# JoeyOL/PytorchDistributed

Measured on AMD Instinct MI355X. Metric: images/sec (whole node) ResNet-50 DDP at 1/2/4/8 MI355X; scaling efficiency, higher is better.
Workload: dtype bf16; 1 GPU; model=resnet50, global_batch=640, per_gpu_batch=640, image_size=224, parallelism=dp1, optimizer=SGD(momentum=0.9, wd=5e-5), fp32 master weights

## Files before the change

### csrc/bindings.cpp

```cpp
#include <torch/extension.h>
#include <c10/hip/HIPStream.h>

#include <map>
#include <mutex>
#include <c10/core/DeviceGuard.h>

#include "pda_kernels.h"
#include "runtime.h"

namespace pda_rt {
void bind_runtime(pybind11::module& m);
}
namespace pda_comm {
void bind_comm(pybind11::module& m);
}

namespace py = pybind11;
using at::Tensor;

namespace {

#define CHECK_HIP_OK(expr)                                                                  \
  do {                                                                                      \
    hipError_t _e = (expr);                                                                 \
// ... 432 lines not shown
  TORCH_CHECK(table.dim() == 3 && table.size(1) == 2 && table.size(2) == C && table.is_contiguous());
  if (relu) {
    TORCH_CHECK(bits.has_value() || ss.has_value(), "relu backward needs the bit mask or scale/shift");
    if (bits.has_value()) {
      check_gpu(*bits, "bits");
      TORCH_CHECK(bits->scalar_type() == at::kByte && bits->is_contiguous() && bits->numel() * 8 == x.numel());
    } else {
      check_f32(*ss, "ss");
      TORCH_CHECK(ss->numel() == 2 * C);
    }
  }
  check_f32(mean, "mean");
  check_f32(invstd, "invstd");
  const float* gf;
  const pda::bf16_t* gb;
  bn_param_ptrs(gamma, &gf, &gb, C);
  c10::DeviceGuard g(x.device());
  Tensor dx = at::empty_like(x);
  Tensor dres = want_dres ? at::empty_like(x) : Tensor();
  const auto pdt = gamma.has_value() ? gamma->scalar_type() : at::kFloat;
  Tensor dgamma = dgamma_out.has_value() ? *dgamma_out : at::empty({C}, x.options().dtype(pdt));
  Tensor dbeta = dbeta_out.has_value() ? *dbeta_out : at::empty({C}, x.options().dtype(pdt));
  TORCH_CHECK(dgamma.numel() == C && dbeta.numel() == C && dgamma.scalar_type() == pdt && dbeta.scalar_type() == pdt);
  const bool pb = pdt == at::kBFloat16;
  Tensor coef = at::empty({3 * C}, x.options().dtype(at::kFloat));
  CHECK_HIP_OK(pda::bn_bwd_table(bp(dy), bp(x), (relu && bits.has_value()) ? bits->data_ptr<uint8_t>() : nullptr,
                                 (relu && !bits.has_value()) ? ss->data_ptr<float>() : nullptr, M, C,
                                 mean.data_ptr<float>(), invstd.data_ptr<float>(), gf, gb, relu, bpm(dx),
                                 want_dres ? bpm(dres) : nullptr, pb ? nullptr : dgamma.data_ptr<float>(),
                                 pb ? bpm(dgamma) : nullptr, pb ? nullptr : dbeta.data_ptr<float>(),
                                 pb ? bpm(dbeta) : nullptr, table.data_ptr<float>(), (int)table.size(0),
                                 coef.data_ptr<float>(), stream_of(x)));
  return {dx, dres, dgamma, dbeta};
}

std::vector<Tensor> maxpool_fwd(Tensor x, int64_t k, int64_t s, int64_t pad) {
  check_bf16(x, "x");
  TORCH_CHECK(x.dim() == 4, "x must be [N,H,W,C]");
  const int N = x.size(0), H = x.size(1), W = x.size(2), C = x.size(3);
  TORCH_CHECK(C % 8 == 0 && k * k <= 255);
  const int P = (H + 2 * pad - k) / s + 1, Q = (W + 2 * pad - k) / s + 1;
  c10::DeviceGuard g(x.device());
  Tensor y = at::empty({N, P, Q, C}, x.options());
  Tensor idx = at::empty({N, P, Q, C}, x.options().dtype(at::kByte));
  CHECK_HIP_OK(pda::maxpool2d_fwd(bp(x), bpm(y), idx.data_ptr<uint8_t>(), N, H, W, C, P, Q, k, s, pad, stream_of(x)));
  return {y, idx};
}

std::vector<Tensor> bn_relu_maxpool_fwd(Tensor x, Tensor table, Tensor shift, c10::optional<Tensor> gamma,
                                        c10::optional<Tensor> beta, Tensor running_mean, Tensor running_var,
                                        c10::optional<Tensor> num_batches, double momentum, double eps, int64_t k,
                                        int64_t s, int64_t pad) {
  check_bf16(x, "x");
  TORCH_CHECK(x.dim() == 4 && x.is_contiguous(), "x must be a contiguous [N,H,W,C] tensor");
  const int N = x.size(0), H = x.size(1), W = x.size(2), C = x.size(3);
  TORCH_CHECK(C % 8 == 0 && C <= 2048 && k * k <= 255);
  check_f32(table, "table");
  check_f32(shift, "shift");
  check_f32(running_mean, "running_mean");
  check_f32(running_var, "running_var");
  TORCH_CHECK(shift.numel() == C && table.numel() % (2 * C) == 0 && table.numel() > 0 && table.is_contiguous(),
              "table must be [R, 2, C]");
  const int P = (H + 2 * pad - k) / s + 1, Q = (W + 2 * pad - k) / s + 1;
  c10::DeviceGuard g(x.device());
  auto fo = x.options().dtype(at::kFloat);
  Tensor stats = at::empty({4, C}, fo);
// ... 1176 lines not shown
  TORCH_CHECK(x.dim() == 4 && x.is_contiguous());
  const int N = x.size(0), HW = x.size(1) * x.size(2), C = x.size(3);
  c10::DeviceGuard g(x.device());
  Tensor y = at::empty({N, C}, x.options());
  CHECK_HIP_OK(pda::avgpool_f32_fwd(x.data_ptr<float>(), y.data_ptr<float>(), N, HW, C, stream_of(x)));
  return y;
}

Tensor avgpool_f32_bwd(Tensor dy, int64_t H, int64_t W) {
  check_f32(dy, "dy");
  TORCH_CHECK(dy.dim() == 2 && dy.is_contiguous());
  const int N = dy.size(0), C = dy.size(1);
  c10::DeviceGuard g(dy.device());
  Tensor dx = at::empty({N, H, W, C}, dy.options());
  CHECK_HIP_OK(pda::avgpool_f32_bwd(dy.data_ptr<float>(), dx.data_ptr<float>(), N, H * W, C, stream_of(dy)));
  return dx;
}

PYBIND11_MODULE(_C, m) {
  m.def("stream_create", &stream_create, py::arg("device"), py::arg("priority"));
  m.def("stream_priority_range", &stream_priority_range, py::arg("device"));
  m.def("stream_create_cumask", &stream_create_cumask, py::arg("device"), py::arg("ncu"), py::arg("invert") = false);
  m.doc() = "pytorchdistributed_amd native layer: CDNA4 HIP kernels + C++ runtime";
  m.def("sgd_step", &sgd_step);
  m.def("adam_step", &adam_step);
  m.def("grad_norm", &grad_norm);
  m.def("cast_scale", &cast_scale);
  m.def("ce_fwd", &ce_fwd);
  m.def("ce_bwd", &ce_bwd);
  m.def("bn_fwd_train", &bn_fwd_train);
  m.def("bn_fwd_eval", &bn_fwd_eval);
  m.def("bn_bwd", &bn_bwd);
  m.def("bn_bwd_table", &bn_bwd_table);
  m.def("set_bn_bwd_fused_max_c", &set_bn_bwd_fused_max_c);
  m.def("set_dgrad_stream", [](int64_t m) { pda::set_dgrad_stream((int)m); });
  m.def("set_fwd_stream", [](int64_t m) { pda::set_fwd_stream((int)m); });
  m.def("set_attn_bwd_fused", [](int64_t m) { pda::attention_bwd_fused_mode() = (int)m; });
  m.def("attn_bwd_fused_mode", []() { return (int64_t)pda::attention_bwd_fused_mode(); });
  m.def("bn_bwd_fused_max_c", []() { return bn_bwd_fused_max_c(); });
  m.def("maxpool_fwd", &maxpool_fwd);
  m.def("bn_relu_maxpool_fwd", &bn_relu_maxpool_fwd);
  m.def("stem_pool_bn_bwd", &stem_pool_bn_bwd);
  m.def("stem_pool_bn_bwd_ok", &stem_pool_bn_bwd_ok);
  m.def("stem_s2d", &stem_s2d);
  m.def("maxpool_bwd", &maxpool_bwd);
  m.def("avgpool_fwd", &avgpool_fwd);
  m.def("avgpool_bwd", &avgpool_bwd);
  m.def("fill_random", &fill_random);
  m.def("fill_randint", &fill_randint);
  m.def("gemm", &gemm);
  m.def("gemm_act", &gemm_act);
  m.def("gemm_wgrad_db", &gemm_wgrad_db);
  m.def("gemm_pp_lab", &gemm_pp_lab);
  m.def("set_gemm_paths", &pda::set_gemm_paths,
        "force a GEMM kernel path: wide=-1 env default, 0 off, 1 auto, 2 force", pybind11::arg("wide"));
  m.def("set_gemm_pp", &pda::set_gemm_pp,
        "pipelined 256x256 kernel for plain wide GEMMs: -1 env default (PDA_GEMM_PP), 0 off, 1 on",
        pybind11::arg("on"));
  m.def("set_splitk_fixup", &pda::set_splitk_fixup,
        "split-K weight gradients reduced by the GEMM's last split per tile: -1 env default (PDA_SPLITK_FIXUP, "
        "off), 0 separate reduce launch, 1 on",
        pybind11::arg("on"));
  m.def("conv_fwd", &conv_fwd, py::arg("x"), py::arg("w"), py::arg("stride"), py::arg("pad"), py::arg("dil"),
        py::arg("bias") = py::none(), py::arg("relu") = false, py::arg("out_f32") = false);
  m.def("split_bf16", &split_bf16, py::arg("x"), py::arg("nseg"), py::arg("lo_mask"), py::arg("stack"));
  m.def("bn_f32_fwd_train", &bn_f32_fwd_train);
// ... 67 lines not shown
```

### csrc/include/pda_kernels.h

```cpp
#pragma once
#include <hip/hip_runtime.h>
#include <stdint.h>

namespace pda {
typedef uint16_t bf16_t;

struct AttnParams {
  const bf16_t *q, *k, *v;
  bf16_t* o;
  float* lse;
  int64_t q_sb, q_st, q_sh, k_sb, k_st, k_sh, v_sb, v_st, v_sh, o_sb, o_st, o_sh;
  int B, T, Hq, Hkv, D, causal;
  float scale;
  const float *rope_cos, *rope_sin;
  const bf16_t* dout;
  int64_t do_sb, do_st, do_sh;
  float* delta;
  bf16_t *dq, *dk, *dv;
  int64_t dq_sb, dq_st, dq_sh, dk_sb, dk_st, dk_sh, dv_sb, dv_st, dv_sh;
  float* dkv_part;
  float* dq_acc;
};

constexpr int kXgmiMaxRanks = 8;
// ... 138 lines not shown
                     void* C, bool c_f32, int64_t ldc, int64_t M, int64_t N, int64_t K, const void* bias,
                     bool bias_f32, bool relu, float* slab, bool allow_split, hipStream_t st);
hipError_t gemm_bf16_wgrad_db(const bf16_t* dy, int64_t ld_dy, const bf16_t* x, int64_t ld_x, void* dw, bool dw_f32,
                              int64_t ldc, int64_t M, int64_t N, int64_t K, void* db, bool db_bf16, float* slab,
                              float* rs_scratch, hipStream_t st, int* db_done);
hipError_t gemm_bf16_act(const bf16_t* A, bool a_kmajor, int64_t lda, const bf16_t* B, bool b_kmajor, int64_t ldb,
                         bf16_t* C, int64_t ldc, int64_t M, int64_t N, int64_t K, const void* bias, bool bias_f32,
                         int act, bf16_t* act_aux, hipStream_t st);
int64_t conv_slab_floats(int mode, int N, int H, int W, int C, int Cout, int R, int S, int P, int Q);
hipError_t conv2d_fwd(const bf16_t* x, const bf16_t* w, void* y, bool y_f32, int N, int H, int W, int C, int Cout,
                      int R, int S, int P, int Q, int stride, int pad, int dil, const void* bias, bool bias_f32,
                      bool relu, float* stats, const float* stats_shift, int stats_rows, hipStream_t st);
bool conv_dgrad_needs_wt(int R, int S, int stride, int pad);
bool conv_dgrad_1x1_wt(int R, int S, int stride, int pad, int C, int Cout);
struct BnBwdStats {
  const bf16_t* z;
  const float* ss;
  const uint8_t* bits;
  const float* mean;
  float* table;
  int rows;
  const bf16_t* z2;
  const float* mean2;
  float* table2;
};
hipError_t conv2d_dgrad(const bf16_t* dy, const bf16_t* w, const bf16_t* wt, void* dx, bool dx_f32, int N, int H, int W,
                        int C, int Cout, int R, int S, int P, int Q, int stride, int pad, int dil, const bf16_t* addend,
                        const uint8_t* addend_bits, hipStream_t st, const BnBwdStats* bst = nullptr);
void set_dgrad_stream(int mode);
void set_fwd_stream(int mode);
hipError_t conv2d_wgrad(const bf16_t* dy, const bf16_t* x, void* dw, bool dw_f32, int N, int H, int W, int C,
                        int Cout, int R, int S, int P, int Q, int stride, int pad, int dil, float* slab,
                        hipStream_t st);
hipError_t conv_weight_transpose(const bf16_t* w, bf16_t* wt, int Cout, int R, int S, int Cin, int stride, int pad,
                                 int dil, hipStream_t st);


hipError_t act_fwd(const void* x, void* y, bool bf16, int64_t n, int op, hipStream_t st);
hipError_t act_bwd(const void* dy, const void* ref, void* dx, bool bf16, int64_t n, int op, hipStream_t st);
hipError_t swiglu_fwd(const void* gu, void* y, bool bf16, int64_t rows, int64_t F, hipStream_t st);
hipError_t swiglu_bwd(const void* dy, const void* gu, void* dgu, bool bf16, int64_t rows, int64_t F, hipStream_t st);
hipError_t colsum_unaligned(const void* x, bool bf16, float* out, int64_t rows, int64_t cols, hipStream_t st);

hipError_t gemm_pp_lab(const bf16_t* A, bool a_kmajor, int64_t lda, const bf16_t* B, bool b_kmajor, int64_t ldb,
                       bf16_t* C, int64_t ldc, int64_t M, int64_t N, int64_t K, const bf16_t* bias, int variant,
                       hipStream_t st);

hipError_t simt_gemm(const void* A, int a_dt, int64_t sam, int64_t sak, const void* B, int b_dt, int64_t sbk,
                     int64_t sbn, void* C, int c_dt, int64_t scm, int64_t scn, int64_t M, int64_t N, int64_t K,
                     const float* bias, bool relu, float beta, hipStream_t st);

hipError_t add_rownorm_fwd(const bf16_t* x, const bf16_t* r, const bf16_t* gamma, const bf16_t* beta, bf16_t* h,
                           bf16_t* y, int64_t rows, int64_t D, float eps, bool rms, hipStream_t st,
                           float* mean = nullptr, float* rstd = nullptr);
hipError_t rownorm_fwd(const void* x, bool x_bf16, const void* gamma, const void* beta, bool p_bf16, void* y,
                       float* mean, float* rstd, int64_t rows, int64_t D, float eps, bool rms, hipStream_t st);
hipError_t rownorm_bwd(const void* dy, const void* x, bool x_bf16, const void* gamma, bool p_bf16, const float* mean,
                       const float* rstd, void* dx, void* dgamma, void* dbeta, bool dparam_bf16, int64_t rows,
                       int64_t D, bool rms, float* ws, hipStream_t st, const void* addend = nullptr);
hipError_t colsum(const void* x, bool bf16, void* out, bool out_bf16, int64_t rows, int64_t cols, float* ws,
                  hipStream_t st);
int64_t colreduce_ws_floats(int64_t rows, int64_t D, int nout);

hipError_t attention_fwd(const AttnParams& p, hipStream_t st);
hipError_t attention_bwd(const AttnParams& p, hipStream_t st);
int64_t attention_bwd_ws_floats(int B, int T, int Hq, int Hkv, int D, bool rope);
// ... 72 lines not shown
```

### csrc/kernels/batchnorm.hip

```cpp
#include "pda_common.h"
#include "pda_kernels.h"

#include <cstdlib>

namespace pda {
namespace {

constexpr int kThreads = 256;
constexpr int kMaxC = 2048;

struct BnGeom {
  int cv;
  int cols;
  int rpi;
  int gy;
  int64_t rpb;
  int nrb;
};

BnGeom bn_geom(int64_t M, int64_t C) {
  BnGeom g;
  g.cv = (int)(C / 8);
  if (g.cv >= kThreads) {
    g.cols = kThreads;
// ... 1128 lines not shown
  int ns = lds_tables_forced() ? 0 : wave_sets((int)(C / 8));
  if (ns == 3 || ns > 4) ns = 0;
  const int grid = ns ? wave_grid(M * C / 8) : ew_grid(M * C / 8);
  const size_t lds = 5 * (size_t)C * sizeof(float);
#define BWD_APPLY(MK, DR)                                                                                        \
  do {                                                                                                           \
    if (ns == 1) bn_bwd_apply_wave_kernel<MK, DR, 1><<<grid, kThreads, 0, st>>>(dy, x, y, ss, M, (int)C, coef, dx, dres); \
    else if (ns == 2) bn_bwd_apply_wave_kernel<MK, DR, 2><<<grid, kThreads, 0, st>>>(dy, x, y, ss, M, (int)C, coef, dx, dres); \
    else if (ns == 4) bn_bwd_apply_wave_kernel<MK, DR, 4><<<grid, kThreads, 0, st>>>(dy, x, y, ss, M, (int)C, coef, dx, dres); \
    else bn_bwd_apply_kernel<MK, DR><<<grid, kThreads, lds, st>>>(dy, x, y, ss, M, (int)C, coef, dx, dres);     \
  } while (0)
  if (mask == 0) { if (dres) BWD_APPLY(0, true); else BWD_APPLY(0, false); }
  else if (mask == 1) { if (dres) BWD_APPLY(1, true); else BWD_APPLY(1, false); }
  else if (mask == 2) { if (dres) BWD_APPLY(2, true); else BWD_APPLY(2, false); }
  else { if (dres) BWD_APPLY(3, true); else BWD_APPLY(3, false); }
#undef BWD_APPLY
  return hipGetLastError();
}

hipError_t bn_bwd_table(const bf16_t* dy, const bf16_t* x, const uint8_t* relu_bits, const float* ss, int64_t M,
                        int64_t C, const float* save_mean, const float* save_invstd, const float* gamma_f,
                        const bf16_t* gamma_b, bool relu, bf16_t* dx, bf16_t* dres, float* dgamma_f, bf16_t* dgamma_b,
                        float* dbeta_f, bf16_t* dbeta_b, float* table, int rows, float* coef, hipStream_t st) {
  if (C > kMaxC || C % 8 || rows < 1 || !table) return hipErrorInvalidValue;
  if (relu && !ss && !relu_bits) return hipErrorInvalidValue;
  bn_bwd_finalize_kernel<true><<<(unsigned)((C + 63) / 64), kFinThreads, 0, st>>>(
      table, rows, M, (int)C, save_mean, save_invstd, gamma_f, gamma_b, dgamma_f, dgamma_b, dbeta_f, dbeta_b, coef);
  PDA_CHECK_HIP(hipGetLastError());
  const int mask = !relu ? 0 : (relu_bits ? 3 : 2);
  const bf16_t* y = mask == 3 ? reinterpret_cast<const bf16_t*>(relu_bits) : nullptr;
  return bwd_apply(dy, x, y, ss, M, C, coef, dx, dres, mask, st);
}

bool bn_bwd_dual_ok(int64_t C) {
  if (C % 8 || C > kMaxC || lds_tables_forced()) return false;
  const int ns = wave_sets((int)(C / 8));
  return ns == 1 || ns == 2;
}

hipError_t bn_bwd_dual(const bf16_t* dy, const uint8_t* relu_bits, int64_t M, int64_t C, const BnBwdSide& a,
                       const BnBwdSide& b, hipStream_t st) {
  if (!bn_bwd_dual_ok(C) || !relu_bits) return hipErrorInvalidValue;
  BnGeom g = bn_geom(M, C);
  float* coef = a.ws + 2 * (int64_t)g.nrb * C;
  float* coef2 = b.ws + 2 * (int64_t)g.nrb * C;
  const bool tables = a.table && b.table;
  if ((a.table != nullptr) != (b.table != nullptr) || (tables && (a.rows < 1 || b.rows < 1))) return hipErrorInvalidValue;
  if (!tables) {
    bn_bwd_reduce_dual_kernel<<<dim3(g.nrb, g.gy), kThreads, 0, st>>>(dy, a.x, b.x, relu_bits, a.mean, b.mean, M,
                                                                     (int)C, g.cols, g.rpi, g.rpb, a.ws, b.ws);
    PDA_CHECK_HIP(hipGetLastError());
  }
  const BnBwdSide* sides[2] = {&a, &b};
  float* coefs[2] = {coef, coef2};
  for (int i = 0; i < 2; ++i) {
    const BnBwdSide& p = *sides[i];
    if (tables)
      bn_bwd_finalize_kernel<true><<<(unsigned)((C + 63) / 64), kFinThreads, 0, st>>>(
          p.table, p.rows, M, (int)C, p.mean, p.invstd, p.gamma_f, p.gamma_b, p.dgamma_f, p.dgamma_b, p.dbeta_f,
          p.dbeta_b, coefs[i]);
    else
      bn_bwd_finalize_kernel<false><<<(unsigned)((C + 63) / 64), kFinThreads, 0, st>>>(
          p.ws, g.nrb, M, (int)C, p.mean, p.invstd, p.gamma_f, p.gamma_b, p.dgamma_f, p.dgamma_b, p.dbeta_f,
          p.dbeta_b, coefs[i]);
    PDA_CHECK_HIP(hipGetLastError());
  }
// ... 38 lines not shown
```

### pytorchdistributed_amd/ops/conv.py

```python
from __future__ import annotations

import os

import torch
import torch.nn.functional as F

from .._native import C
from ..parallel.flat import grad_target
from . import streams as _streams
from .grad_join import MaskedGrad


_SIDE_1X1 = os.environ.get("PDA_WGRAD_SIDE_1X1", "1") == "1"


def _ref_conv(x, w, stride, padding, dilation, bias=None):
    y = F.conv2d(x.permute(0, 3, 1, 2), w.permute(0, 3, 1, 2), bias, stride, padding, dilation)
    return y.permute(0, 2, 3, 1).contiguous()


class _Conv2dFn(torch.autograd.Function):
    @staticmethod
    def forward(ctx, x, w, bias, stride, padding, dilation, relu, join, bnb=None):
        x = x.contiguous()
        w = w.contiguous()
        y = C().conv_fwd(x, w, stride, padding, dilation, bias, relu)
        ctx.save_for_backward(x, w, y if relu else None)
        ctx.cfg = (stride, padding, dilation, relu, bias is not None)
        ctx.wparam = w
        ctx.join = join
        ctx.bnb = bnb
        return y

    @staticmethod
    def backward(ctx, dy):
        return _Conv2dFn._backward(ctx, dy)

    @staticmethod
    def _backward(ctx, dy):
        x, w, y = ctx.saved_tensors
        stride, padding, dilation, relu, has_bias = ctx.cfg
        dy = dy.contiguous()
        if relu:
            dy = C().relu_bwd(dy, y)
        dx = dw = db = None
        if ctx.needs_input_grad[0]:
            join = ctx.join
            if join is not None and not join.is_last():
                join.stash(C().conv_dgrad(dy, w, x.shape[1], x.shape[2], stride, padding, dilation, None))
            else:
                bnb = getattr(ctx, "bnb", None)
                join_last = join is not None and join.is_last()
                addend = join.take() if join is not None else None
                bits = None
                if isinstance(addend, MaskedGrad):
                    addend, bits = addend.grad, addend.bits
                kw = {}
                if bnb is not None and bnb.usable(join_last, join is not None, stride, addend) and \
                        bnb.z.shape == x.shape:
                    kw = bnb.dgrad_kwargs()
                dx = C().conv_dgrad(dy, w, x.shape[1], x.shape[2], stride, padding, dilation, addend, bits, **kw)
                if kw:
                    bnb.mark_filled(dx)
        ctx.bnb = None
        if ctx.needs_input_grad[1]:
            target = grad_target(ctx.wparam)
            args = (dy, x, w.shape[1], w.shape[2], stride, padding, dilation, w.dtype == torch.float32, target)
            if target is not None and _streams.side_ok(ctx.wparam) and (_SIDE_1X1 or w.shape[1] * w.shape[2] > 1):
                with _streams.wgrad_stream(dy.device, dy, x):
                    dw = C().conv_wgrad(*args)
            else:
                dw = C().conv_wgrad(*args)
        if has_bias and ctx.needs_input_grad[2]:
            db = dy.reshape(-1, dy.shape[-1]).sum(0, dtype=torch.float32).to(dy.dtype)
        return dx, dw, db, None, None, None, None, None, None


class _Conv2dStatsFn(torch.autograd.Function):

    @staticmethod
    def forward(ctx, x, w, stride, padding, dilation, shift, table, join, bnb=None):
        x = x.contiguous()
        w = w.contiguous()
        y = C().conv_fwd_stats(x, w, stride, padding, dilation, shift, table)
        ctx.save_for_backward(x, w, None)
        ctx.cfg = (stride, padding, dilation, False, False)
        ctx.wparam = w
        ctx.join = join
        ctx.bnb = bnb
        return y

    @staticmethod
    def backward(ctx, dy):
        dx, dw, _db, *_ = _Conv2dFn._backward(ctx, dy)
        return dx, dw, None, None, None, None, None, None, None


def conv2d_bn_stats(x: torch.Tensor, weight: torch.Tensor, stride: int = 1, padding: int = 0, dilation: int = 1,
                    shift: torch.Tensor = None, table: torch.Tensor = None, grad_join=None):
    if weight.shape[-1] != x.shape[-1]:
        weight = F.pad(weight, (0, x.shape[-1] - weight.shape[-1]))
    return _Conv2dStatsFn.apply(x, weight, stride, padding, dilation, shift, table, grad_join,
                                getattr(x, "_pda_bnb", None))


def conv2d(x: torch.Tensor, weight: torch.Tensor, bias=None, stride: int = 1, padding: int = 0, dilation: int = 1,
           relu: bool = False, grad_join=None) -> torch.Tensor:
    if x.is_cuda:
        if weight.shape[-1] != x.shape[-1]:
            weight = F.pad(weight, (0, x.shape[-1] - weight.shape[-1]))
        if x.dtype == torch.float32:
            from . import fp32

            return fp32.conv2d(x, weight, bias, stride, padding, dilation, relu)
        return _Conv2dFn.apply(x, weight, bias, stride, padding, dilation, relu, grad_join,
                               getattr(x, "_pda_bnb", None))
    if weight.shape[-1] != x.shape[-1]:
        x = x[..., : weight.shape[-1]]
    y = _ref_conv(x, weight, stride, padding, dilation, bias)
    return torch.relu(y) if relu else y
```

### pytorchdistributed_amd/ops/grad_join.py

```python
from __future__ import annotations

from typing import Optional, Union

import torch


class MaskedGrad:

    __slots__ = ("grad", "bits")

    def __init__(self, grad: torch.Tensor, bits: torch.Tensor):
        self.grad, self.bits = grad, bits

    def materialize(self) -> torch.Tensor:
        shifts = torch.arange(8, device=self.bits.device, dtype=torch.uint8)
        mask = ((self.bits.reshape(-1, 1) >> shifts) & 1).bool().reshape(self.grad.shape)
        return torch.where(mask, self.grad, torch.zeros((), dtype=self.grad.dtype, device=self.grad.device))


def _dense(g):
    return g.materialize() if isinstance(g, MaskedGrad) else g


class GradJoin:
# ... 52 lines not shown
        self.filled = False
        if (dx is not None and dy.data_ptr() == dx.data_ptr() and dy.shape == dx.shape and dy._version == ver):
            return True
        self.table.zero_()
        if self.table2 is not None:
            self.table2.zero_()
        return False

    @property
    def filled(self) -> bool:
        return self.token[0][0]

    @filled.setter
    def filled(self, v: bool):
        for t in self.token:
            t[0] = bool(v)

    def usable(self, join_last: bool, has_join: bool, stride: int, addend) -> bool:
        if self.z is None:
            return False
        if self.needs_join and not (has_join and join_last):
            return False
        return stride == 1 or addend is None

    def dgrad_kwargs(self) -> dict:
        kw = dict(bst_z=self.z, bst_mean=self.mean, bst_table=self.table)
        if self.bits is not None:
            kw["bst_bits"] = self.bits
        else:
            kw["bst_ss"] = self.ss
        if self.z2 is not None:
            kw.update(bst_z2=self.z2, bst_mean2=self.mean2, bst_table2=self.table2)
        return kw
```

### pytorchdistributed_amd/ops/norm.py

```python
from __future__ import annotations

import os

import torch
import torch.nn.functional as F

from .._native import C
from ..parallel.flat import grad_target
from .grad_join import BnBwdStats, MaskedGrad


class _BatchNormFn(torch.autograd.Function):
    @staticmethod
    def forward(ctx, x, gamma, beta, residual, running_mean, running_var, training, momentum, eps, relu, join,
                table=None, shift=None, num_batches=None, bwd_table=None):
        x = x.contiguous()
        if residual is not None:
            residual = residual.contiguous()
        ss = bits = None
        want_bits = relu and residual is not None
        if training and table is not None:
            y, mean, invstd, ss, bits = C().bn_fwd_train_sums(x, table, shift, residual, gamma, beta, running_mean,
                                                              running_var, momentum, eps, relu, want_bits, num_batches)
        elif training:
            y, mean, invstd, ss, bits = C().bn_fwd_train(x, residual, gamma, beta, running_mean, running_var,
                                                         momentum, eps, relu, want_bits, num_batches)
        else:
            y = C().bn_fwd_eval(x, residual, gamma, beta, running_mean, running_var, eps, relu)
            mean = running_mean
            invstd = torch.rsqrt(running_var + eps)
        ctx.save_for_backward(x, bits if want_bits else None, ss if (relu and not want_bits) else None, mean, invstd,
                              gamma)
        ctx.cfg = (relu, residual is not None, training)
        ctx.beta = beta
        ctx.join = join
        ctx.bnb = None
        if bwd_table is not None and training and relu and (bits is not None or ss is not None):
            table_, token = bwd_table
            ctx.bnb = BnBwdStats(x, ss if bits is None else None, bits, mean, table_, residual is not None, token)
        return y

    @staticmethod
    def backward(ctx, dy):
        x, bits, ss, mean, invstd, gamma = ctx.saved_tensors
        relu, has_res, training = ctx.cfg
        if not training:
            raise NotImplementedError("backward through eval-mode BatchNorm is not supported")
        tg = grad_target(gamma) if gamma is not None and ctx.needs_input_grad[1] else None
        tb = grad_target(ctx.beta) if ctx.beta is not None and ctx.needs_input_grad[2] else None
        if (tg is None) != (tb is None):
            tg = tb = None
        dy = dy.contiguous()
        masked = has_res and ctx.join is not None and bits is not None and not ctx.join.is_last()
        bnb = ctx.bnb
        if bnb is not None and bnb.take_if_matches(dy):
            dx, dres, dgamma, dbeta = C().bn_bwd_table(dy, x, bits, ss if bits is None else None, mean, invstd, gamma,
                                                       relu, has_res and not masked, bnb.table, tg, tb)
        else:
            dx, dres, dgamma, dbeta = C().bn_bwd(dy, x, bits, ss, mean, invstd, gamma, relu, has_res and not masked,
                                                 tg, tb)
        ctx.bnb = None
        dg = dgamma if gamma is not None and ctx.needs_input_grad[1] else None
        db = dbeta if ctx.needs_input_grad[2] else None
        if masked:
            ctx.join.stash(MaskedGrad(dy, bits))
            dres = None
        elif has_res and ctx.join is not None:
            dres = ctx.join.contribute(dres)
        return dx, dg, db, (dres if has_res else None), None, None, None, None, None, None, None, None, None, None, None


def _param_targets(ctx, gamma, beta, ig, ib):
    tg = grad_target(gamma) if gamma is not None and ctx.needs_input_grad[ig] else None
    tb = grad_target(beta) if beta is not None and ctx.needs_input_grad[ib] else None
    return (None, None) if (tg is None) != (tb is None) else (tg, tb)


_DUAL_BWD = os.environ.get("PDA_DUAL_BN_BWD", "1") == "1"


class _DualBatchNormFn(torch.autograd.Function):

    @staticmethod
    def forward(ctx, x, gamma, beta, x2, gamma2, beta2, rm, rv, rm2, rv2, table, shift, table2, shift2, nbt, nbt2,
                momentum, eps, bwd_tables=None):
        x, x2 = x.contiguous(), x2.contiguous()
        y, bits, mean, invstd, mean2, invstd2 = C().bn_fwd_train_sums_dual(
            x, table, shift, gamma, beta, rm, rv, nbt, x2, table2, shift2, gamma2, beta2, rm2, rv2, nbt2, momentum,
            eps)
        ctx.save_for_backward(x, x2, bits, mean, invstd, mean2, invstd2, gamma, gamma2)
        ctx.betas = (beta, beta2)
        ctx.bnb = None
        if bwd_tables is not None:
            (bt1, tok), (bt2, tok2) = bwd_tables
            ctx.bnb = BnBwdStats(x, None, bits, mean, bt1, True, (tok, tok2), second=(x2, mean2, bt2))
        return y

    @staticmethod
    def backward(ctx, dy):
        x, x2, bits, mean, invstd, mean2, invstd2, gamma, gamma2 = ctx.saved_tensors
        beta, beta2 = ctx.betas
        dy = dy.contiguous()
# ... 32 lines not shown
        m = x.numel() // x.shape[-1]
        bt = (bn.bwd_table(x.device, m), bn2.bwd_table(x.device, m))
    y = _DualBatchNormFn.apply(x, bn.weight, bn.bias, x2, bn2.weight, bn2.bias, bn.running_mean, bn.running_var,
                               bn2.running_mean, bn2.running_var, t1, s1, t2, s2, bn.num_batches_tracked,
                               bn2.num_batches_tracked, bn.momentum, bn.eps, bt)
    if bt is not None and y.grad_fn is not None and getattr(y.grad_fn, "bnb", None) is not None:
        y._pda_bnb = y.grad_fn.bnb
    return y


def _ref_batch_norm(x, gamma, beta, residual, running_mean, running_var, training, momentum, eps, relu):
    C_ = x.shape[-1]
    xf = x.reshape(-1, C_)
    g = gamma.float() if gamma is not None else None
    b = beta.float() if beta is not None else None
    y = F.batch_norm(xf.float(), running_mean, running_var, g, b, training, momentum, eps)
    y = y.reshape(x.shape)
    if residual is not None:
        y = y + residual.float()
    if relu:
        y = torch.relu(y)
    return y.to(x.dtype)


_BWD_EPILOGUE = os.environ.get("PDA_BN_BWD_EPILOGUE", "1") == "1"


def batch_norm(x, gamma, beta, running_mean=None, running_var=None, training=True, momentum=0.1, eps=1e-5,
               residual=None, relu=False, residual_join=None, stats=None, num_batches_tracked=None, bwd_table=None):
    if x.is_cuda and x.dtype == torch.bfloat16:
        table, shift = stats if stats is not None else (None, None)
        bt = bwd_table if (_BWD_EPILOGUE and training and torch.is_grad_enabled()) else None
        y = _BatchNormFn.apply(x, gamma, beta, residual, running_mean, running_var, training, momentum, eps,
                               relu, residual_join, table, shift, num_batches_tracked if training else None, bt)
        if bt is not None and y.grad_fn is not None:
            bnb = getattr(y.grad_fn, "bnb", None)
            if bnb is not None:
                y._pda_bnb = bnb
        return y
    if x.is_cuda and x.dtype == torch.float32 and x.shape[-1] % 4 == 0 and residual_join is None:
        from . import fp32

        return fp32.batch_norm(x, gamma, beta, running_mean, running_var, training, momentum, eps, residual, relu,
                               num_batches_tracked)
    if training and num_batches_tracked is not None:
        num_batches_tracked.add_(1)
    return _ref_batch_norm(x, gamma, beta, residual, running_mean, running_var, training, momentum, eps, relu)


def _param_grad_slots(ctx, gi: int):
    gamma, beta = ctx.params
    ng = ctx.needs_input_grad
    tg = grad_target(gamma) if ng[gi] else None
    tb = grad_target(beta) if (beta is not None and ng[gi + 1]) else None
    if beta is not None and (tg is None) != (tb is None):
        for p, t in ((gamma, tg), (beta, tb)):
            if t is not None:
                p._pda_claimed = False
        tg = tb = None
    return tg, tb


class _RowNormFn(torch.autograd.Function):
    @staticmethod
    def forward(ctx, x, gamma, beta, eps, rms):
        x = x.contiguous()
        y, mean, rstd = C().rownorm_fwd(x, gamma.contiguous(), beta, eps, rms)
# ... 70 lines not shown
```

Before: 10320 images/sec.

## Fuse bottleneck BN3 backward apply with following 1x1 conv dgrad and BN2 stats

Adds a streaming kernel that applies the BN backward coefficients (with ReLU mask) to produce dz3, immediately multiplies it by the 1x1 conv weight held in LDS via MFMA to produce the conv's input gradient, and accumulates the next BN's backward reduction statistics in the same pass. A Python handoff object passes the precomputed dgrad from the BN backward to the conv backward, so the conv skips its own dgrad launch. This removes a round trip of dz3 through HBM and a separate dgrad GEMM plus stats pass, at the cost of a fragile cross-op handoff with version checks and a fallback path. It applies only to K=256/N=64 and K=512/N=128 shapes with enough rows, and only when the residual is masked.

```diff
diff --git a/csrc/bindings.cpp b/csrc/bindings.cpp
--- a/csrc/bindings.cpp
+++ b/csrc/bindings.cpp
@@ -488,6 +488,75 @@
                                  pb ? bpm(dbeta) : nullptr, table.data_ptr<float>(), (int)table.size(0),
                                  coef.data_ptr<float>(), stream_of(x)));
   return {dx, dres, dgamma, dbeta};
+}
+
+Tensor conv_dgrad(Tensor dy, Tensor w, int64_t H, int64_t W, int64_t stride, int64_t pad, int64_t dil,
+                  c10::optional<Tensor> addend, c10::optional<Tensor> addend_bits, bool out_f32,
+                  c10::optional<Tensor> bst_z, c10::optional<Tensor> bst_ss, c10::optional<Tensor> bst_bits,
+                  c10::optional<Tensor> bst_mean, c10::optional<Tensor> bst_table, c10::optional<Tensor> bst_z2,
+                  c10::optional<Tensor> bst_mean2, c10::optional<Tensor> bst_table2);
+
+std::vector<Tensor> bn_bwd_table_dgrad(Tensor dy, Tensor x, c10::optional<Tensor> bits, c10::optional<Tensor> ss,
+                                       Tensor mean, Tensor invstd, c10::optional<Tensor> gamma, bool relu,
+                                       bool want_dres, Tensor table, c10::optional<Tensor> dgamma_out,
+                                       c10::optional<Tensor> dbeta_out, Tensor w, Tensor bst_z, Tensor bst_ss,
+                                       Tensor bst_mean, Tensor bst_table) {
+  TORCH_CHECK(!want_dres, "bn_bwd_table_dgrad: the residual gradient is handed over as (dy, bits)");
+  check_bf16(x, "x");
+  check_bf16(w, "w");
+  TORCH_CHECK(x.dim() == 4 && w.dim() == 4 && w.size(1) == 1 && w.size(2) == 1 && w.size(0) == x.size(3) &&
+                  w.is_contiguous(),
+              "bn_bwd_table_dgrad: x must be [N, H, W, C] and w the [C, 1, 1, N] weight of the conv that produced it");
+  const int64_t C = x.size(-1), M = x.numel() / C, N = w.size(3);
+  if (!(relu && bits.has_value() && pda::bn_bwd_dgrad_stream_ok(M, C, N))) {
+    auto r = bn_bwd_table(dy, x, bits, ss, mean, invstd, gamma, relu, false, table, dgamma_out, dbeta_out);
+    Tensor da = conv_dgrad(r[0], w, x.size(1), x.size(2), 1, 0, 1, c10::nullopt, c10::nullopt, false, bst_z, bst_ss,
+                           c10::nullopt, bst_mean, bst_table, c10::nullopt, c10::nullopt, c10::nullopt);
+    return {r[0], da, r[2], r[3]};
+  }
+  check_bf16(dy, "dy");
+  TORCH_CHECK(dy.sizes() == x.sizes());
+  check_f32(table, "table");
+  TORCH_CHECK(table.dim() == 3 && table.size(1) == 2 && table.size(2) == C && table.is_contiguous());
+  check_gpu(*bits, "bits");
+  TORCH_CHECK(bits->scalar_type() == at::kByte && bits->is_contiguous() && bits->numel() * 8 == x.numel());
+  check_f32(mean, "mean");
+  check_f32(invstd, "invstd");
+  TORCH_CHECK(mean.numel() == C && invstd.numel() == C);
+  check_bf16(bst_z, "bst_z");
+  check_f32(bst_ss, "bst_ss");
+  check_f32(bst_mean, "bst_mean");
+  check_f32(bst_table, "bst_table");
+  TORCH_CHECK(bst_z.dim() == 4 && bst_z.size(0) == x.size(0) && bst_z.size(1) == x.size(1) &&
+                  bst_z.size(2) == x.size(2) && bst_z.size(3) == N && bst_z.is_contiguous(),
+              "bst_z must have the conv input's shape");
+  TORCH_CHECK(bst_ss.numel() == 2 * N && bst_mean.numel() == N && bst_table.dim() == 3 && bst_table.size(1) == 2 &&
+                  bst_table.size(2) == N && bst_table.is_contiguous(),
+              "bst_table must be a contiguous [R, 2, N] fp32 table");
+  const float* gf;
+  const pda::bf16_t* gb;
+  bn_param_ptrs(gamma, &gf, &gb, C);
+  c10::DeviceGuard g(x.device());
+  Tensor dx = at::empty_like(x);
+  Tensor da = at::empty_like(bst_z);
+  const auto pdt = gamma.has_value() ? gamma->scalar_type() : at::kFloat;
+  Tensor dgamma = dgamma_out.has_value() ? *dgamma_out : at::empty({C}, x.options().dtype(pdt));
+  Tensor dbeta = dbeta_out.has_value() ? *dbeta_out : at::empty({C}, x.options().dtype(pdt));
+  TORCH_CHECK(dgamma.numel() == C && dbeta.numel() == C && dgamma.scalar_type() == pdt && dbeta.scalar_type() == pdt);
+  const bool pb = pdt == at::kBFloat16;
+  Tensor coef = at::empty({3 * C}, x.options().dtype(at::kFloat));
+  pda::BnBwdStats bn2{};
+  bn2.z = bp(bst_z);
+  bn2.ss = bst_ss.data_ptr<float>();
+  bn2.mean = bst_mean.data_ptr<float>();
+  bn2.table = bst_table.data_ptr<float>();
+  bn2.rows = (int)bst_table.size(0);
+  CHECK_HIP_OK(pda::bn_bwd_table_dgrad(bp(dy), bp(x), bits->data_ptr<uint8_t>(), M, C, mean.data_ptr<float>(),
+                                       invstd.data_ptr<float>(), gf, gb, bpm(dx), pb ? nullptr : dgamma.data_ptr<float>(),
+                                       pb ? bpm(dgamma) : nullptr, pb ? nullptr : dbeta.data_ptr<float>(),
+                                       pb ? bpm(dbeta) : nullptr, table.data_ptr<float>(), (int)table.size(0),
+                                       coef.data_ptr<float>(), bp(w), N, bpm(da), bn2, stream_of(x)));
+  return {dx, da, dgamma, dbeta};
 }
 
 std::vector<Tensor> maxpool_fwd(Tensor x, int64_t k, int64_t s, int64_t pad) {
@@ -1730,6 +1799,11 @@
   m.def("bn_fwd_eval", &bn_fwd_eval);
   m.def("bn_bwd", &bn_bwd);
   m.def("bn_bwd_table", &bn_bwd_table);
+  m.def("bn_bwd_table_dgrad", &bn_bwd_table_dgrad);
+  m.def("bn_bwd_dgrad_ok",
+        [](int64_t M, int64_t K, int64_t N) { return pda::bn_bwd_dgrad_stream_ok(M, K, N); });
+  m.def("set_bn_bwd_dgrad", [](int64_t m, int64_t wgs) { pda::set_bn_bwd_dgrad((int)m, (int)wgs); }, py::arg("mode"),
+        py::arg("max_workgroups") = 0);
   m.def("set_bn_bwd_fused_max_c", &set_bn_bwd_fused_max_c);
   m.def("set_dgrad_stream", [](int64_t m) { pda::set_dgrad_stream((int)m); });
   m.def("set_fwd_stream", [](int64_t m) { pda::set_fwd_stream((int)m); });
diff --git a/csrc/include/pda_kernels.h b/csrc/include/pda_kernels.h
--- a/csrc/include/pda_kernels.h
+++ b/csrc/include/pda_kernels.h
@@ -194,6 +194,16 @@
 hipError_t conv2d_wgrad(const bf16_t* dy, const bf16_t* x, void* dw, bool dw_f32, int N, int H, int W, int C,
                         int Cout, int R, int S, int P, int Q, int stride, int pad, int dil, float* slab,
                         hipStream_t st);
+bool bn_bwd_dgrad_stream_ok(int64_t M, int64_t K, int64_t N);
+hipError_t bn_bwd_dgrad_stream(const bf16_t* dout, const bf16_t* z3, const uint8_t* bits, const float* coef,
+                               const bf16_t* w, bf16_t* dz3, bf16_t* da2, int64_t M, int64_t K, int64_t N,
+                               const BnBwdStats& bn2, hipStream_t st);
+void set_bn_bwd_dgrad(int mode, int max_workgroups = 0);
+hipError_t bn_bwd_table_dgrad(const bf16_t* dy, const bf16_t* x, const uint8_t* relu_bits, int64_t M, int64_t C,
+                              const float* save_mean, const float* save_invstd, const float* gamma_f,
+                              const bf16_t* gamma_b, bf16_t* dx, float* dgamma_f, bf16_t* dgamma_b, float* dbeta_f,
+                              bf16_t* dbeta_b, float* table, int rows, float* coef, const bf16_t* w, int64_t N,
+                              bf16_t* da2, const BnBwdStats& bn2, hipStream_t st);
 hipError_t conv_weight_transpose(const bf16_t* w, bf16_t* wt, int Cout, int R, int S, int Cin, int stride, int pad,
                                  int dil, hipStream_t st);
 
diff --git a/csrc/kernels/batchnorm.hip b/csrc/kernels/batchnorm.hip
--- a/csrc/kernels/batchnorm.hip
+++ b/csrc/kernels/batchnorm.hip
@@ -1184,6 +1184,18 @@
   return bwd_apply(dy, x, y, ss, M, C, coef, dx, dres, mask, st);
 }
 
+hipError_t bn_bwd_table_dgrad(const bf16_t* dy, const bf16_t* x, const uint8_t* relu_bits, int64_t M, int64_t C,
+                              const float* save_mean, const float* save_invstd, const float* gamma_f,
+                              const bf16_t* gamma_b, bf16_t* dx, float* dgamma_f, bf16_t* dgamma_b, float* dbeta_f,
+                              bf16_t* dbeta_b, float* table, int rows, float* coef, const bf16_t* w, int64_t N,
+                              bf16_t* da2, const BnBwdStats& bn2, hipStream_t st) {
+  if (rows < 1 || !table || !relu_bits || !bn_bwd_dgrad_stream_ok(M, C, N)) return hipErrorInvalidValue;
+  bn_bwd_finalize_kernel<true><<<(unsigned)((C + 63) / 64), kFinThreads, 0, st>>>(
+      table, rows, M, (int)C, save_mean, save_invstd, gamma_f, gamma_b, dgamma_f, dgamma_b, dbeta_f, dbeta_b, coef);
+  PDA_CHECK_HIP(hipGetLastError());
+  return bn_bwd_dgrad_stream(dy, x, relu_bits, coef, w, dx, da2, M, C, N, bn2, st);
+}
+
 bool bn_bwd_dual_ok(int64_t C) {
   if (C % 8 || C > kMaxC || lds_tables_forced()) return false;
   const int ns = wave_sets((int)(C / 8));
diff --git a/csrc/kernels/bn_bwd_dgrad_stream.hip b/csrc/kernels/bn_bwd_dgrad_stream.hip
--- /dev/null
+++ b/csrc/kernels/bn_bwd_dgrad_stream.hip
@@ -0,0 +1,261 @@
+#include "pda_common.h"
+#include "pda_kernels.h"
+
+#include <cstdlib>
+
+namespace pda {
+namespace {
+
+typedef __bf16 bdbf16x8 __attribute__((ext_vector_type(8)));
+
+constexpr int BD_NT = 512;
+constexpr int BD_NW = BD_NT / 64;
+constexpr int BD_KC = 4;
+constexpr int BD_PITCH = 72;
+constexpr int BD_CUS = 256;
+
+struct BDArgs {
+  const bf16_t* dout;
+  const bf16_t* z3;
+  const uint8_t* bits;
+  const float* coef;
+  const bf16_t* w;
+  bf16_t* dz3;
+  bf16_t* da2;
+  const bf16_t* z2;
+  const float* ss2;
+  const float* mean2;
+  float* table2;
+  int rows2;
+  int64_t M;
+  int64_t ntiles;
+};
+
+template <int K, int N>
+__global__ void __launch_bounds__(BD_NT) bn_bwd_dgrad_stream_kernel(BDArgs a) {
+  constexpr int KS = K / 32;
+  constexpr int NCH = KS / BD_KC;
+  constexpr int NJ = N / 16;
+  constexpr int NH = N / 64;
+  constexpr int WFRAG_BYTES = K * N * 2;
+  static_assert(2 * BD_NW * N * 4 <= WFRAG_BYTES, "the flush scratch reuses the weight fragments");
+  extern __shared__ __attribute__((aligned(16))) char smem[];
+  u16x8* wfrag = reinterpret_cast<u16x8*>(smem);
+  float* s_co = reinterpret_cast<float*>(smem + WFRAG_BYTES);
+  float* s_par = s_co + 3 * K;
+  bf16_t* patches = reinterpret_cast<bf16_t*>(s_par + 3 * N);
+  const int tid = threadIdx.x, lane = tid & 63;
+  const int wid = __builtin_amdgcn_readfirstlane(tid >> 6);
+  const int g = lane >> 4, r16 = lane & 15;
+  bf16_t* stg = patches + wid * (16 * BD_PITCH);
+
+  for (int f = tid; f < NJ * KS * 64; f += BD_NT) {
+    const int l = f & 63, kk = (f >> 6) % KS, j = f / (64 * KS);
+    const bf16_t* p = a.w + (int64_t)(32 * kk + 8 * (l >> 4)) * N + 16 * j + (l & 15);
+    u16x8 v;
+#pragma unroll
+    for (int i = 0; i < 8; ++i) v[i] = p[(int64_t)i * N];
+    wfrag[f] = v;
+  }
+  for (int c = tid; c < 3 * K; c += BD_NT) s_co[c] = a.coef[c];
+  for (int c = tid; c < N; c += BD_NT) {
+    s_par[c] = a.mean2[c];
+    s_par[N + c] = a.ss2[c];
+    s_par[2 * N + c] = a.ss2[N + c];
+  }
+  __syncthreads();
+
+  struct Chunk {
+    u16x8 dy[BD_KC], z[BD_KC];
+    uint32_t mb[BD_KC];
+  };
+  auto load = [&](int64_t t, int c, Chunk& p) {
+    const int64_t m = t * 16 + r16;
+    const int64_t base = (m < a.M ? m : 0) * K + 128 * c + 8 * g;
+#pragma unroll
+    for (int kk = 0; kk < BD_KC; ++kk) {
+      p.dy[kk] = *reinterpret_cast<const u16x8*>(a.dout + base + 32 * kk);
+      p.z[kk] = *reinterpret_cast<const u16x8*>(a.z3 + base + 32 * kk);
+      p.mb[kk] = a.bits[(base + 32 * kk) >> 3];
+    }
+  };
+
+  float st1[NH][8], st2[NH][8];
+#pragma unroll
+  for (int h = 0; h < NH; ++h)
+#pragma unroll
+    for (int q = 0; q < 8; ++q) st1[h][q] = st2[h][q] = 0.f;
+
+  const int64_t stride = (int64_t)gridDim.x * BD_NW;
+  int64_t t = (int64_t)blockIdx.x * BD_NW + wid;
+  Chunk cur;
+  if (t < a.ntiles) load(t, 0, cur);
+  for (; t < a.ntiles; t += stride) {
+    const int64_t m = t * 16 + r16;
+    const bool row_ok = m < a.M;
+    f32x4 acc[NJ];
+#pragma unroll
+    for (int j = 0; j < NJ; ++j) acc[j] = f32x4{0.f, 0.f, 0.f, 0.f};
+    u16x8 zc[NH][2];
+#pragma unroll 1
+    for (int c = 0; c < NCH; ++c) {
+      Chunk nxt;
+      if (c + 1 < NCH) load(t, c + 1, nxt);
+      else if (t + stride < a.ntiles) load(t + stride, 0, nxt);
+      if (c == NCH - 1) {
+#pragma unroll
+        for (int h = 0; h < NH; ++h)
+#pragma unroll
+          for (int u = 0; u < 2; ++u) {
+            const int64_t me = t * 16 + (lane >> 3) + 8 * u;
+            zc[h][u] = *reinterpret_cast<const u16x8*>(a.z2 + (me < a.M ? me : 0) * N + 64 * h + 8 * (lane & 7));
+          }
+      }
+#pragma unroll
+      for (int kk = 0; kk < BD_KC; ++kk) {
+        const int c0 = 128 * c + 32 * kk + 8 * g;
+        float cA[8], cB[8], cC[8];
+        load8(s_co + c0, cA);
+        load8(s_co + K + c0, cB);
+        load8(s_co + 2 * K + c0, cC);
+        u16x8 o;
+#pragma unroll
+        for (int i = 0; i < 8; ++i) {
+          const float gv = (cur.mb[kk] >> i) & 1u ? bf2f(cur.dy[kk][i]) : 0.f;
+          o[i] = f2bf(fmaf(cA[i], gv, fmaf(cB[i], bf2f(cur.z[kk][i]), cC[i])));
+        }
+        if (row_ok) __builtin_nontemporal_store(o, reinterpret_cast<u16x8*>(a.dz3 + m * K + c0));
+        const bdbf16x8 af = __builtin_bit_cast(bdbf16x8, o);
+#pragma unroll
+        for (int j = 0; j < NJ; ++j) {
+          const bdbf16x8 wf = __builtin_bit_cast(bdbf16x8, wfrag[(j * KS + BD_KC * c + kk) * 64 + lane]);
+          acc[j] = __builtin_amdgcn_mfma_f32_16x16x32_bf16(wf, af, acc[j], 0, 0, 0);
+        }
+      }
+      cur = nxt;
+    }
+#pragma unroll
+    for (int h = 0; h < NH; ++h) {
+#pragma unroll
+      for (int jj = 0; jj < 4; ++jj) {
+        u16x4 o;
+#pragma unroll
+        for (int q = 0; q < 4; ++q) o[q] = f2bf(acc[4 * h + jj][q]);
+        *reinterpret_cast<u16x4*>(stg + r16 * BD_PITCH + 16 * jj + 4 * g) = o;
+      }
+      __builtin_amdgcn_fence(__ATOMIC_RELEASE, "wavefront");
+      __builtin_amdgcn_wave_barrier();
+      __builtin_amdgcn_fence(__ATOMIC_ACQUIRE, "wavefront");
+      const int nc = 64 * h + 8 * (lane & 7);
+      float kmu[8], scl[8], shf[8];
+      load8(s_par + nc, kmu);
+      load8(s_par + N + nc, scl);
+      load8(s_par + 2 * N + nc, shf);
+#pragma unroll
+      for (int u = 0; u < 2; ++u) {
+        const int r = (lane >> 3) + 8 * u;
+        const int64_t me = t * 16 + r;
+        const u16x8 o = *reinterpret_cast<const u16x8*>(stg + r * BD_PITCH + 8 * (lane & 7));
+        if (me >= a.M) continue;
+#pragma unroll
+        for (int q = 0; q < 8; ++q) {
+          const float zf = bf2f(zc[h][u][q]);
+          const float gv = fmaf(zf, scl[q], shf[q]) > 0.f ? bf2f(o[q]) : 0.f;
+          st1[h][q] += gv;
+          st2[h][q] = fmaf(gv, zf - kmu[q], st2[h][q]);
+        }
+        *reinterpret_cast<u16x8*>(a.da2 + me * N + nc) = o;
+      }
+      __builtin_amdgcn_fence(__ATOMIC_RELEASE, "wavefront");
+      __builtin_amdgcn_wave_barrier();
+      __builtin_amdgcn_fence(__ATOMIC_ACQUIRE, "wavefront");
+    }
+  }
+
+#pragma unroll
+  for (int off = 8; off < 64; off <<= 1)
+#pragma unroll
+    for (int h = 0; h < NH; ++h)
+#pragma unroll
+      for (int q = 0; q < 8; ++q) {
+        st1[h][q] += __shfl_xor(st1[h][q], off, 64);
+        st2[h][q] += __shfl_xor(st2[h][q], off, 64);
+      }
+  __syncthreads();
+  float* red = reinterpret_cast<float*>(smem);
+  if (lane < 8) {
+#pragma unroll
+    for (int h = 0; h < NH; ++h)
+#pragma unroll
+      for (int q = 0; q < 8; ++q) {
+        red[(wid * 2 + 0) * N + 64 * h + 8 * lane + q] = st1[h][q];
+        red[(wid * 2 + 1) * N + 64 * h + 8 * lane + q] = st2[h][q];
+      }
+  }
+  __syncthreads();
+  if (tid < 2 * N) {
+    float s = 0.f;
+#pragma unroll
+    for (int w = 0; w < BD_NW; ++w) s += red[w * 2 * N + tid];
+    unsafeAtomicAdd(a.table2 + (int64_t)(blockIdx.x % (unsigned)a.rows2) * 2 * N + tid, s);
+  }
+}
+
+int g_mode_override = -1;
+int g_wgs_override = 0;
+
+int fuse_mode() {
+  static const int m = [] {
+    const char* s = getenv("PDA_BN3_DGRAD_FUSE");
+    return s ? atoi(s) : 1;
+  }();
+  return g_mode_override >= 0 ? g_mode_override : m;
+}
+
+bool deterministic_env() {
+  const char* s = getenv("PDA_DETERMINISTIC");
+  return s != nullptr && s[0] == '1';
+}
+
+template <int K, int N>
+hipError_t launch(const BDArgs& a, unsigned grid, hipStream_t st) {
+  constexpr size_t lds = (size_t)K * N * 2 + (3 * K + 3 * N) * sizeof(float) + BD_NW * 16 * BD_PITCH * 2;
+  static_assert(lds <= 160 * 1024, "one workgroup's LDS");
+  static const hipError_t attr = hipFuncSetAttribute(reinterpret_cast<const void*>(&bn_bwd_dgrad_stream_kernel<K, N>),
+                                                     hipFuncAttributeMaxDynamicSharedMemorySize, (int)lds);
+  PDA_CHECK_HIP(attr);
+  bn_bwd_dgrad_stream_kernel<K, N><<<grid, BD_NT, lds, st>>>(a);
+  return hipGetLastError();
+}
+
+}
+
+void set_bn_bwd_dgrad(int mode, int max_workgroups) {
+  g_mode_override = mode;
+  g_wgs_override = max_workgroups > 0 ? max_workgroups : 0;
+}
+
+bool bn_bwd_dgrad_stream_ok(int64_t M, int64_t K, int64_t N) {
+  const int mode = fuse_mode();
+  if (mode <= 0 || M <= 0) return false;
+  if (!((K == 256 && N == 64) || (K == 512 && N == 128))) return false;
+  if (mode == 1 && M < (int64_t)16 * BD_NW * BD_CUS) return false;
+  return true;
+}
+
+hipError_t bn_bwd_dgrad_stream(const bf16_t* dout, const bf16_t* z3, const uint8_t* bits, const float* coef,
+                               const bf16_t* w, bf16_t* dz3, bf16_t* da2, int64_t M, int64_t K, int64_t N,
+                               const BnBwdStats& bn2, hipStream_t st) {
+  if (!bn_bwd_dgrad_stream_ok(M, K, N)) return hipErrorInvalidValue;
+  if (!dout || !z3 || !bits || !coef || !w || !dz3 || !da2) return hipErrorInvalidValue;
+  if (!bn2.z || !bn2.ss || !bn2.mean || !bn2.table || bn2.rows < 1 || bn2.bits || bn2.z2) return hipErrorInvalidValue;
+  BDArgs a{dout, z3, bits, coef, w, dz3, da2, bn2.z, bn2.ss, bn2.mean, bn2.table, bn2.rows, M, (M + 15) / 16};
+  int64_t gx = (a.ntiles + BD_NW - 1) / BD_NW;
+  if (gx > BD_CUS) gx = BD_CUS;
+  if (g_wgs_override > 0 && gx > g_wgs_override) gx = g_wgs_override;
+  if ((deterministic_env() || M <= (int64_t)256 * bn2.rows) && gx > bn2.rows) gx = bn2.rows;
+  if (K == 256) return launch<256, 64>(a, (unsigned)gx, st);
+  return launch<512, 128>(a, (unsigned)gx, st);
+}
+
+}
diff --git a/pytorchdistributed_amd/ops/conv.py b/pytorchdistributed_amd/ops/conv.py
--- a/pytorchdistributed_amd/ops/conv.py
+++ b/pytorchdistributed_amd/ops/conv.py
@@ -8,7 +8,7 @@
 from .._native import C
 from ..parallel.flat import grad_target
 from . import streams as _streams
-from .grad_join import MaskedGrad
+from .grad_join import ConvDgradHandoff, MaskedGrad
 
 
 _SIDE_1X1 = os.environ.get("PDA_WGRAD_SIDE_1X1", "1") == "1"
@@ -44,7 +44,10 @@
         if relu:
             dy = C().relu_bwd(dy, y)
         dx = dw = db = None
-        if ctx.needs_input_grad[0]:
+        dgh = getattr(ctx, "dgh", None)
+        if dgh is not None:
+            dx = dgh.take_if_matches(dy)
+        if dx is None and ctx.needs_input_grad[0]:
             join = ctx.join
             if join is not None and not join.is_last():
                 join.stash(C().conv_dgrad(dy, w, x.shape[1], x.shape[2], stride, padding, dilation, None))
@@ -88,6 +91,10 @@
         ctx.wparam = w
         ctx.join = join
         ctx.bnb = bnb
+        ctx.dgh = None
+        if (bnb is not None and join is None and ctx.needs_input_grad[0] and w.shape[1] == 1 and w.shape[2] == 1
+                and stride == 1 and padding == 0 and bnb.z.shape == x.shape):
+            ctx.dgh = ConvDgradHandoff(w, bnb)
         return y
 
     @staticmethod
@@ -100,8 +107,12 @@
                     shift: torch.Tensor = None, table: torch.Tensor = None, grad_join=None):
     if weight.shape[-1] != x.shape[-1]:
         weight = F.pad(weight, (0, x.shape[-1] - weight.shape[-1]))
-    return _Conv2dStatsFn.apply(x, weight, stride, padding, dilation, shift, table, grad_join,
-                                getattr(x, "_pda_bnb", None))
+    y = _Conv2dStatsFn.apply(x, weight, stride, padding, dilation, shift, table, grad_join,
+                             getattr(x, "_pda_bnb", None))
+    dgh = getattr(y.grad_fn, "dgh", None) if y.grad_fn is not None else None
+    if dgh is not None:
+        y._pda_dgh = dgh
+    return y
 
 
 def conv2d(x: torch.Tensor, weight: torch.Tensor, bias=None, stride: int = 1, padding: int = 0, dilation: int = 1,
diff --git a/pytorchdistributed_amd/ops/grad_join.py b/pytorchdistributed_amd/ops/grad_join.py
--- a/pytorchdistributed_amd/ops/grad_join.py
+++ b/pytorchdistributed_amd/ops/grad_join.py
@@ -108,3 +108,38 @@
         if self.z2 is not None:
             kw.update(bst_z2=self.z2, bst_mean2=self.mean2, bst_table2=self.table2)
         return kw
+
+    def discard(self):
+        self.dx, self.dx_ver = None, -1
+        self.filled = False
+        self.table.zero_()
+        if self.table2 is not None:
+            self.table2.zero_()
+
+
+class ConvDgradHandoff:
+
+    __slots__ = ("w", "bnb", "dz", "dz_ver", "dx")
+
+    def __init__(self, w: torch.Tensor, bnb: "BnBwdStats"):
+        self.w, self.bnb = w, bnb
+        self.dz, self.dz_ver, self.dx = None, -1, None
+
+    def ready(self) -> bool:
+        b = self.bnb
+        return (b is not None and b.z is not None and b.ss is not None and b.bits is None and b.z2 is None
+                and not b.needs_join and self.dx is None)
+
+    def deposit(self, dz: torch.Tensor, dx: torch.Tensor):
+        self.dz, self.dz_ver, self.dx = dz, dz._version, dx
+        self.bnb.mark_filled(dx)
+
+    def take_if_matches(self, dy: torch.Tensor) -> Optional[torch.Tensor]:
+        dz, ver, dx = self.dz, self.dz_ver, self.dx
+        self.dz, self.dz_ver, self.dx = None, -1, None
+        if dx is None:
+            return None
+        if dy.data_ptr() == dz.data_ptr() and dy.shape == dz.shape and dy._version == ver:
+            return dx
+        self.bnb.discard()
+        return None
diff --git a/pytorchdistributed_amd/ops/norm.py b/pytorchdistributed_amd/ops/norm.py
--- a/pytorchdistributed_amd/ops/norm.py
+++ b/pytorchdistributed_amd/ops/norm.py
@@ -13,7 +13,7 @@
 class _BatchNormFn(torch.autograd.Function):
     @staticmethod
     def forward(ctx, x, gamma, beta, residual, running_mean, running_var, training, momentum, eps, relu, join,
-                table=None, shift=None, num_batches=None, bwd_table=None):
+                table=None, shift=None, num_batches=None, bwd_table=None, dgh=None):
         x = x.contiguous()
         if residual is not None:
             residual = residual.contiguous()
@@ -38,6 +38,7 @@
         if bwd_table is not None and training and relu and (bits is not None or ss is not None):
             table_, token = bwd_table
             ctx.bnb = BnBwdStats(x, ss if bits is None else None, bits, mean, table_, residual is not None, token)
+        ctx.dgh = dgh if (training and want_bits and dgh is not None and x.dim() == 4) else None
         return y
 
     @staticmethod
@@ -53,9 +54,19 @@
         dy = dy.contiguous()
         masked = has_res and ctx.join is not None and bits is not None and not ctx.join.is_last()
         bnb = ctx.bnb
+        dgh = ctx.dgh
         if bnb is not None and bnb.take_if_matches(dy):
-            dx, dres, dgamma, dbeta = C().bn_bwd_table(dy, x, bits, ss if bits is None else None, mean, invstd, gamma,
-                                                       relu, has_res and not masked, bnb.table, tg, tb)
+            if (dgh is not None and masked and dgh.ready()
+                    and C().bn_bwd_dgrad_ok(x.numel() // x.shape[-1], x.shape[-1], dgh.w.shape[-1])):
+                b2 = dgh.bnb
+                dx, da, dgamma, dbeta = C().bn_bwd_table_dgrad(dy, x, bits, None, mean, invstd, gamma, relu, False,
+                                                               bnb.table, tg, tb, dgh.w, b2.z, b2.ss, b2.mean,
+                                                               b2.table)
+                dgh.deposit(dx, da)
+                dres = None
+            else:
+                dx, dres, dgamma, dbeta = C().bn_bwd_table(dy, x, bits, ss if bits is None else None, mean, invstd,
+                                                           gamma, relu, has_res and not masked, bnb.table, tg, tb)
         else:
             dx, dres, dgamma, dbeta = C().bn_bwd(dy, x, bits, ss, mean, invstd, gamma, relu, has_res and not masked,
                                                  tg, tb)
@@ -67,7 +78,7 @@
             dres = None
         elif has_res and ctx.join is not None:
             dres = ctx.join.contribute(dres)
-        return dx, dg, db, (dres if has_res else None), None, None, None, None, None, None, None, None, None, None, None
+        return (dx, dg, db, (dres if has_res else None)) + (None,) * 12
 
 
 def _param_targets(ctx, gamma, beta, ig, ib):
@@ -166,7 +177,8 @@
         table, shift = stats if stats is not None else (None, None)
         bt = bwd_table if (_BWD_EPILOGUE and training and torch.is_grad_enabled()) else None
         y = _BatchNormFn.apply(x, gamma, beta, residual, running_mean, running_var, training, momentum, eps,
-                               relu, residual_join, table, shift, num_batches_tracked if training else None, bt)
+                               relu, residual_join, table, shift, num_batches_tracked if training else None, bt,
+                               getattr(x, "_pda_dgh", None) if bt is not None else None)
         if bt is not None and y.grad_fn is not None:
             bnb = getattr(y.grad_fn, "bnb", None)
             if bnb is not None:
```

Result: slower. 10170 images/sec (-1.5%).
